# embedded-software-laboratory/p-dmpc

Hardware: NVIDIA B200
Metric: vehicle-plans/sec (higher is better)
Workload: dtype f64

## Files before the change

include/pdmpc_b200.h:

```cpp
#ifndef PDMPC_B200_H
#define PDMPC_B200_H

#include <stddef.h>
#include <stdint.h>

#ifdef __cplusplus
extern "C" {
#endif

#define PDMPC_ABI_VERSION 2

#define PDMPC_AREA_STRIDE 8
#define PDMPC_MAX_HP 16
#define PDMPC_MAX_TRIMS 128
#define PDMPC_MAX_JOINT 4
#define PDMPC_MAX_PRED_LANELETS 8

enum pdmpc_status {
    PDMPC_OK = 0,
    PDMPC_ERR_BAD_INPUT = 1,
    PDMPC_ERR_CUDA = 2,
    PDMPC_ERR_CAPACITY = 3,
    PDMPC_ERR_NO_MPA = 4,
    PDMPC_ERR_ALLOC = 5
// ... 80 lines not shown

int pdmpc_create(int device_id, pdmpc_handle **out);
int pdmpc_destroy(pdmpc_handle *h);
const char *pdmpc_last_error(const pdmpc_handle *h);
int pdmpc_abi_version(void);
int pdmpc_get_hp(const pdmpc_handle *h);

int pdmpc_set_node_capacity(pdmpc_handle *h, int32_t max_nodes_per_search);

int pdmpc_set_variant(pdmpc_handle *h, int32_t variant);

int pdmpc_set_cta_queue(pdmpc_handle *h, int32_t valid_only);

int pdmpc_set_escalation(pdmpc_handle *h, int32_t pops, int32_t short_list_max);

int pdmpc_set_tile_points(pdmpc_handle *h, int32_t points);

int pdmpc_set_cta_heap_smem(pdmpc_handle *h, int32_t entries);

int pdmpc_set_pipeline_chunks(pdmpc_handle *h, int32_t chunks);

int pdmpc_pipeline_bounds(int32_t n_searches, int32_t chunks, int32_t cap, int32_t *bounds, int32_t *n_chunks);

int pdmpc_get_pipeline_timeline(pdmpc_handle *h, int32_t cap, double *host_ms, double *in_ms, double *done_ms, int32_t *n_chunks);

int pdmpc_upload_mpa(pdmpc_handle *h, const pdmpc_mpa_desc *mpa);

int pdmpc_plan_batch(pdmpc_handle *h, const pdmpc_batch_in *in, pdmpc_batch_out *out);

int pdmpc_stage_batch(pdmpc_handle *h, const pdmpc_batch_in *in);
// ... 124 lines not shown
```

p-dmpc_b200/capi.py:

```python
from __future__ import annotations

import ctypes as C
import os
from typing import Optional

import numpy as np

from .mpa import MotionPrimitiveAutomaton
from .records import BatchResult, SearchBatch

_PKG_DIR = os.path.dirname(os.path.abspath(__file__))
LIB_PATH = os.path.join(_PKG_DIR, "csrc", "libpdmpc_b200.so")

PDMPC_OK = 0
PDMPC_ERR_BAD_INPUT = 1
PDMPC_ERR_CUDA = 2
PDMPC_ERR_CAPACITY = 3
PDMPC_ERR_NO_MPA = 4
PDMPC_ERR_ALLOC = 5

EXPORTED_SYMBOLS = (
    "pdmpc_create", "pdmpc_destroy", "pdmpc_last_error", "pdmpc_abi_version",
    "pdmpc_set_node_capacity", "pdmpc_set_variant", "pdmpc_set_tile_points", "pdmpc_set_cta_queue", "pdmpc_set_escalation", "pdmpc_get_hp", "pdmpc_pack_plan_rows", "pdmpc_upload_road", "pdmpc_sample_inputs", "pdmpc_upload_reachable_sets", "pdmpc_assemble_obstacles", "pdmpc_get_pipeline_timeline", "pdmpc_pipeline_bounds", "pdmpc_plan_timestep_from_states", "pdmpc_closed_loop_reset", "pdmpc_plan_timestep_closed_loop", "pdmpc_host_alloc", "pdmpc_host_free",
    "pdmpc_trace_staged", "pdmpc_upload_mpa", "pdmpc_plan_batch", "pdmpc_stage_batch",
    "pdmpc_run_staged", "pdmpc_sync", "pdmpc_fetch_staged", "pdmpc_get_stats", "pdmpc_stream",
    "pdmpc_mcts_plan_batch", "pdmpc_mcts_run_staged", "pdmpc_set_cta_heap_smem", "pdmpc_plan_timestep",
    "pdmpc_set_pipeline_chunks", "pdmpc_measure_fp64_peak", "pdmpc_joint_plan_batch",
)

_p_u8 = C.POINTER(C.c_uint8)
_p_i32 = C.POINTER(C.c_int32)
_p_u64 = C.POINTER(C.c_uint64)
_p_f64 = C.POINTER(C.c_double)


class MpaDesc(C.Structure):
    _fields_ = [
        ("n_trims", C.c_int32), ("Hp", C.c_int32), ("n_edges", C.c_int32),
# ... 180 lines not shown
    lib.pdmpc_get_pipeline_timeline.argtypes = [H, C.c_int32, _p_f64, _p_f64, _p_f64, C.POINTER(C.c_int32)]
    lib.pdmpc_get_pipeline_timeline.restype = C.c_int
    lib.pdmpc_pipeline_bounds.argtypes = [C.c_int32, C.c_int32, C.c_int32, _p_i32, C.POINTER(C.c_int32)]
    lib.pdmpc_pipeline_bounds.restype = C.c_int
    lib.pdmpc_plan_timestep_from_states.argtypes = [H, C.POINTER(TimestepStatesC), C.POINTER(BatchOut)]
    lib.pdmpc_plan_timestep_from_states.restype = C.c_int
    lib.pdmpc_closed_loop_reset.argtypes = [H, C.c_int32, C.c_double, C.c_double]
    lib.pdmpc_closed_loop_reset.restype = C.c_int
    lib.pdmpc_plan_timestep_closed_loop.argtypes = [H, C.POINTER(BatchIn), C.POINTER(TimestepDepsC), _p_i32,
                                                    C.POINTER(C.c_uint8), C.POINTER(BatchOut)]
    lib.pdmpc_plan_timestep_closed_loop.restype = C.c_int
    lib.pdmpc_get_hp.argtypes = [H]
    lib.pdmpc_get_hp.restype = C.c_int
    lib.pdmpc_set_escalation.argtypes = [H, C.c_int32, C.c_int32]
    lib.pdmpc_set_escalation.restype = C.c_int
    lib.pdmpc_set_tile_points.argtypes = [H, C.c_int32]
    lib.pdmpc_set_tile_points.restype = C.c_int
    lib.pdmpc_trace_staged.argtypes = [H, C.c_int32, C.POINTER(C.c_int64), C.c_int64, C.POINTER(C.c_int64)]
    lib.pdmpc_trace_staged.restype = C.c_int
    lib.pdmpc_host_alloc.argtypes = [C.POINTER(C.c_void_p), C.c_size_t]
    lib.pdmpc_host_alloc.restype = C.c_int
    lib.pdmpc_host_free.argtypes = [C.c_void_p]
    lib.pdmpc_host_free.restype = C.c_int
    lib.pdmpc_upload_mpa.argtypes = [H, C.POINTER(MpaDesc)]
    lib.pdmpc_upload_mpa.restype = C.c_int
    lib.pdmpc_plan_batch.argtypes = [H, C.POINTER(BatchIn), C.POINTER(BatchOut)]
    lib.pdmpc_plan_batch.restype = C.c_int
    lib.pdmpc_stage_batch.argtypes = [H, C.POINTER(BatchIn)]
    lib.pdmpc_stage_batch.restype = C.c_int
    lib.pdmpc_run_staged.argtypes = [H]
# ... 160 lines not shown
             "vert_x": np.zeros(vc), "vert_y": np.zeros(vc)}
        ci = CouplingInC(n=n, x=_ptr(x, _p_f64), y=_ptr(y, _p_f64), yaw=_ptr(yaw, _p_f64), speed=_ptr(speed, _p_f64),
                         trim=_ptr(trim, _p_i32), succ_ptr=_ptr(sp, _p_i32), succ_idx=_ptr(si, _p_i32),
                         par_ptr=_ptr(pp, _p_i32), par_idx=_ptr(pi, _p_i32),
                         half_length=float(half_length), half_width=float(half_width))
        oc = ObstaclesOutC(slot_ptr=_ptr(o["slot_ptr"], _p_i32), poly_ptr=_ptr(o["poly_ptr"], _p_i32),
                           vert_x=_ptr(o["vert_x"], _p_f64), vert_y=_ptr(o["vert_y"], _p_f64), poly_capacity=pc, vert_capacity=vc)
        self._check(self.lib.pdmpc_assemble_obstacles(self.h, C.byref(ci), C.byref(oc)))
        o["poly_ptr"] = o["poly_ptr"][: oc.n_polys + 1]
        o["vert_x"], o["vert_y"] = o["vert_x"][: oc.n_verts], o["vert_y"][: oc.n_verts]
        return o

    def set_escalation(self, pops: int, short_list_max: int = -1):
        self._check(self.lib.pdmpc_set_escalation(self.h, int(pops), int(short_list_max)))

    def set_tile_points(self, points: int = 0):
        self._check(self.lib.pdmpc_set_tile_points(self.h, int(points)))

    def trace(self, search: int, cap: int = 1 << 20) -> np.ndarray:
        ids = np.zeros(cap, dtype=np.int64)
        n = C.c_int64()
        self._check(self.lib.pdmpc_trace_staged(self.h, int(search), ids.ctypes.data_as(C.POINTER(C.c_int64)),
                                                cap, C.byref(n)))
        return ids[: min(n.value, cap)].copy()

    def upload_mpa(self, mpa: MotionPrimitiveAutomaton):
        d, keep = mpa_desc(mpa)
        self._check(self.lib.pdmpc_upload_mpa(self.h, C.byref(d)))
        self._mpa_keep = keep
        self._mpa = mpa
# ... 131 lines not shown
```

p-dmpc_b200/csrc/pdmpc_capi.cu:

```cuda
#include <cuda_runtime.h>

#include <algorithm>
#include <cmath>
#include <cstdio>
#include <cstdlib>
#include <cstring>
#include <chrono>
#include <new>
#include <string>
#include <vector>

#include "pdmpc_kernels.cuh"
#include "pdmpc_tiles.cuh"
#include "pdmpc_mcts.cuh"
#include "pdmpc_cta.cuh"
#include "pdmpc_joint.cuh"
#include "pdmpc_inputs.cuh"
#include "pdmpc_fallback.cuh"
#include "pdmpc_obstacles.cuh"

using namespace pdmpc;

namespace {

// ... 27 lines not shown
#ifndef PDMPC_TILE4_PTS
#define PDMPC_TILE4_PTS 256
#endif
constexpr int kTile2Heap = PDMPC_TILE2_HEAP, kTile2Pts = PDMPC_TILE2_PTS, kTile2Ctas = PDMPC_TILE2_CTAS;
constexpr int kTile4Heap = PDMPC_TILE4_HEAP, kTile4Pts = PDMPC_TILE4_PTS, kTile4Ctas = PDMPC_TILE4_CTAS;
#define KERNEL_TILE2 search_tile_kernel<16, kTile2Heap, kTile2Pts, kTile2Ctas>
#define KERNEL_TILE4 search_tile_kernel<8, kTile4Heap, kTile4Pts, kTile4Ctas>
constexpr size_t kTile2Smem = 2 * sizeof(TileSm<kTile2Heap, kTile2Pts>);
constexpr size_t kTile4Smem = 4 * sizeof(TileSm<kTile4Heap, kTile4Pts>);
#ifndef PDMPC_CTA_MASTERS
#define PDMPC_CTA_MASTERS 4
#endif
#ifndef PDMPC_ESCALATE_POPS
#define PDMPC_ESCALATE_POPS 2560
#endif
constexpr int kCtaCheckers = 12;
constexpr int kCtaHeap = 4096, kCtaPts = 512;
constexpr int kCtaMHeap = 1024, kCtaMPts = 256;
constexpr int kCtaMasters = PDMPC_CTA_MASTERS, kCtaMastersDeps = 2;
#define KERNEL_CTA search_cta_kernel<kCtaHeap, kCtaPts, kCtaCheckers, 1, false>
#define KERNEL_CTA_DEPS search_cta_kernel<kCtaHeap, kCtaPts, kCtaCheckers, 1, true>
#define KERNEL_CTAM search_cta_kernel<kCtaMHeap, kCtaMPts, kCtaCheckers, kCtaMasters, false>
#define KERNEL_CTAM_DEPS search_cta_kernel<kCtaMHeap, kCtaMPts, kCtaCheckers, kCtaMastersDeps, true>
using CtaSmemT = CtaSmem<kCtaHeap, kCtaPts, kCtaCheckers, 1, false>;
using CtaDepsSmemT = CtaSmem<kCtaHeap, kCtaPts, kCtaCheckers, 1, true>;
using CtaMSmemT = CtaSmem<kCtaMHeap, kCtaMPts, kCtaCheckers, kCtaMasters, false>;
using CtaMDepsSmemT = CtaSmem<kCtaMHeap, kCtaMPts, kCtaCheckers, kCtaMastersDeps, true>;
static_assert(sizeof(CtaSmemT) <= kSmemLimit && sizeof(CtaDepsSmemT) <= kSmemLimit && sizeof(CtaMSmemT) <= kSmemLimit &&
              sizeof(CtaMDepsSmemT) <= kSmemLimit, "CTA shapes must fit one SM");

// ... 112 lines not shown
    x.a += off; x.b += off; x.cs += off; x.heap += off;
    return x;
}

}

struct pdmpc_handle {
    int device = 0;
    int num_sms = 0;
    int lat_ctas_per_sm = 0;
    int tile_ctas_per_sm[2] = {0, 0};
    int tile_pts_limit = 0;
    int variant_mode = 0;
    int cta_heap_smem = kCtaHeap;
    int escalate_pops = -1;
    int esc_short_list = -1;
    DBuf esc;
    DBuf esc_rows;
    PinnedBuf pin_esc;

    bool cta_valid_only = false;
    bool cta_ok = false;
    bool cta_deps_ok = false;
    DBuf j_veh, j_node, j_heap;
    DBuf d_deps, d_done, d_depx, d_depy, d_depn;
    bool lat_deps_ok = false;
    PinnedBuf pin_deps;
    DepsDev deps{};
    bool deps_staged = false;
    std::vector<int> topo_order;
    cudaStream_t s_in = nullptr, s_out = nullptr, s_comp[7] = {};
// ... 422 lines not shown
    o.n_expanded = reinterpret_cast<int *>(base + h->out_off[2]);
    o.n_pops = reinterpret_cast<int *>(base + h->out_off[3]);
    o.pop_hash = reinterpret_cast<unsigned long long *>(base + h->out_off[4]);
    o.trims = reinterpret_cast<int *>(base + h->out_off[5]);
    o.tree_path = reinterpret_cast<int *>(base + h->out_off[6]);
    o.y_predicted = reinterpret_cast<double *>(base + h->out_off[7]);
    o.g_path = reinterpret_cast<double *>(base + h->out_off[8]);
    o.h_path = reinterpret_cast<double *>(base + h->out_off[9]);
    o.shape_npts = reinterpret_cast<int *>(base + h->out_off[10]);
    o.shape_x = reinterpret_cast<double *>(base + h->out_off[11]);
    o.shape_y = reinterpret_cast<double *>(base + h->out_off[12]);
    o.counters = reinterpret_cast<unsigned long long *>(base + h->out_off[kNumOut]);
    return PDMPC_OK;
}

static void read_counters(pdmpc_handle *h, const unsigned long long counters[16]) {
    h->stats.total_pops = (int64_t)counters[0];
    h->stats.total_nodes = (int64_t)counters[1];
    h->stats.total_obstacle_cols = (int64_t)counters[2];
    if (counters[3]) h->stats.handed_over = (int32_t)counters[3];
    h->stats.escalated = (int32_t)counters[6];
#ifdef PDMPC_PROFILE
    {
#ifdef PDMPC_PROFILE_CHECKER
        static const char *names[8] = {"c:wait_job", "c:tables+place", "c:interx_obstacles", "c:interx_rest", "c:sincos+publish", "-", "-", "c:other"};
#else
        static const char *names[8] = {"setup", "heap_pop", "loads+place", "check", "expand", "heap_push", "wait_children", "loop"};
#endif
        double tot = 0;
        for (int i = 0; i < 8; ++i) tot += (double)counters[8 + i];
        fprintf(stderr, "[pdmpc profile] cycles per pop:");
        for (int i = 0; i < 8; ++i)
            fprintf(stderr, " %s=%.0f", names[i], (double)counters[8 + i] / (double)std::max<unsigned long long>(counters[0], 1));
        fprintf(stderr, " total=%.0f\n", tot / (double)std::max<unsigned long long>(counters[0], 1));
        if (counters[5])
            fprintf(stderr, "[pdmpc profile] checker 0: %.0f cycles per job over %llu jobs\n",
                    (double)counters[4] / (double)counters[5], counters[5]);
    }
#endif
}

static int reserve_polylines(pdmpc_handle *h, int np, int nv, int nl) {
    BatchDev &b = h->batch;
    b.pl_x = b.pl_y = b.ll_x = b.ll_y = nullptr;
    b.pl_xy = b.ll_xy = nullptr;
    if (b.checker != PDMPC_CHECKER_INTERX) return PDMPC_OK;
    CU_TRY(h, h->b_plx.reserve(((size_t)nv + np + 1) * sizeof(double)));
    CU_TRY(h, h->b_ply.reserve(((size_t)nv + np + 1) * sizeof(double)));
    CU_TRY(h, h->b_llx.reserve(((size_t)nl + 2 * b.n + 1) * sizeof(double)));
    CU_TRY(h, h->b_lly.reserve(((size_t)nl + 2 * b.n + 1) * sizeof(double)));
    CU_TRY(h, h->b_plxy.reserve(((size_t)nv + np + 1) * sizeof(double2)));
    CU_TRY(h, h->b_llxy.reserve(((size_t)nl + 2 * b.n + 1) * sizeof(double2)));
    b.pl_x = h->b_plx.as<double>(); b.pl_y = h->b_ply.as<double>();
    b.ll_x = h->b_llx.as<double>(); b.ll_y = h->b_lly.as<double>();
// ... 100 lines not shown
    return stage_finish(h, n, in->checker, in->dt_seconds, dptr, np, nv, nl);
}

static int node_cap(const pdmpc_handle *h) {
    const int cap = h->user_node_cap ? h->user_node_cap : std::min(h->full_tree_nodes + 8, 1 << 20);
    return std::max(std::min(cap, kMaxNodeCap - 1), 64);
}

static bool cta_launchable(const pdmpc_handle *h, bool deps) {
    return (deps ? h->cta_deps_ok : h->cta_ok) && node_cap(h) <= kCtaFlags;
}

static int ensure_arena(pdmpc_handle *h, int slots) {
    const int cap = node_cap(h);
    if (slots <= h->arena_slots && cap == h->arena.cap) return PDMPC_OK;
    slots = std::max(slots, h->arena_slots);
    const size_t tot = (size_t)slots * cap;
    h->arena = ArenaDev{};
    h->arena_slots = 0;
    CU_TRY(h, h->a_a.reserve(tot * sizeof(NodeA)));
    CU_TRY(h, h->a_b.reserve(tot * sizeof(NodeB)));
    CU_TRY(h, h->a_cs.reserve(tot * sizeof(NodeCS)));
    CU_TRY(h, h->a_heap.reserve(tot * sizeof(HEnt)));
    h->arena.a = h->a_a.as<NodeA>();
    h->arena.b = h->a_b.as<NodeB>();
    h->arena.cs = h->a_cs.as<NodeCS>();
    h->arena.heap = h->a_heap.as<HEnt>();
    h->arena.cap = cap;
    h->arena_slots = slots;
    return PDMPC_OK;
}
// ... 25 lines not shown
    else if (shape == kShapeTile4) KERNEL_TILE4<<<grid, kWarp, kTile4Smem, S>>>(h->mpa, bc, h->out, ar, wc, tr, h->tile_pts_limit);
    else KERNEL_LAT<<<grid, kWarp, sizeof(WarpSmem), S>>>(h->mpa, bc, h->out, ar, wc, tr);
    if (cudaGetLastError() != cudaSuccess) return fail(h, PDMPC_ERR_CUDA, "search kernel launch failed");
    h->stats.kernel_launches++;
    return PDMPC_OK;
}

static int escalation_pops(const pdmpc_handle *h, int n) {
    if (h->escalate_pops >= 0) return h->escalate_pops;
    return n >= 300000 ? 4096 : n >= 120000 ? 3072 : PDMPC_ESCALATE_POPS;
}
static bool escalation_on(const pdmpc_handle *h, int shape, int n) {
    return (shape == kShapeTile2 || shape == kShapeTile4) && escalation_pops(h, n) > 0 && cta_launchable(h, false) &&
           n > h->num_sms && h->batch.checker == PDMPC_CHECKER_INTERX;
}

static int escalation_prepare(pdmpc_handle *h, int n, BatchDev *bt, cudaStream_t S) {
    CU_TRY(h, h->esc.reserve(((size_t)n + 4) * sizeof(int)));
    CU_TRY(h, cudaMemsetAsync(h->esc.p, 0, 4 * sizeof(int), S));
    CU_TRY(h, cudaMemsetAsync(h->esc.as<int>() + 4, 0xff, (size_t)n * sizeof(int), S));
    bt->pop_limit = escalation_pops(h, n);
    bt->esc_count = h->esc.as<unsigned>();
    bt->esc_done = h->esc.as<unsigned>() + 1;
    bt->esc_list = h->esc.as<int>() + 4;
    return PDMPC_OK;
}

static int launch_escalated(pdmpc_handle *h, const ArenaDev &ar, int producers, cudaStream_t S) {
    BatchDev be = h->batch;
    be.order = nullptr;
    be.esc_count = h->esc.as<unsigned>();
    be.esc_done = h->esc.as<unsigned>() + 1;
    be.esc_list = h->esc.as<int>() + 4;
    be.esc_producers = (unsigned)producers;
    const int fast = h->cta_valid_only ? 1 : 0;
    unsigned *wc = h->work_counter.as<unsigned>();
    be.esc_gate_lo = 0u; be.esc_gate_hi = (unsigned)(h->esc_short_list >= 0 ? h->esc_short_list : 3 * h->num_sms);
    KERNEL_CTA<<<h->num_sms, CtaShape<1, kCtaCheckers>::kThreads, sizeof(CtaSmemT), S>>>(
        h->mpa, be, h->out, ar, wc + 1, h->cta_heap_smem, fast, DepsDev{});
    be.esc_gate_lo = be.esc_gate_hi; be.esc_gate_hi = 0xffffffffu;
    KERNEL_CTAM<<<h->num_sms, CtaShape<kCtaMasters, kCtaCheckers>::kThreads, sizeof(CtaMSmemT), S>>>(
        h->mpa, be, h->out, ar, wc + 2, h->cta_heap_smem, fast, DepsDev{});
    if (cudaGetLastError() != cudaSuccess) return fail(h, PDMPC_ERR_CUDA, "escalation kernel launch failed");
    h->stats.kernel_launches += 2;
    return PDMPC_OK;
}

static int launch_search(pdmpc_handle *h, const TraceDev &tr) {
    const int n = h->batch.n;
    CU_TRY(h, cudaSetDevice(h->device));
    CU_TRY(h, cudaMemsetAsync(h->out.counters, 0, kCounterBytes, h->stream));
    CU_TRY(h, cudaMemsetAsync(h->work_counter.p, 0, 4 * sizeof(unsigned), h->stream));
    h->stats.handed_over = 0;
    h->stats.escalated = 0;
    h->stats.shape = 0;
    h->batch.hash_valid_only = h->cta_valid_only ? 1 : 0;
    if (n == 0) return PDMPC_OK;
    int shape = h->variant_mode;
    if (shape == kShapeAuto && n <= h->num_sms && tr.search < 0) shape = kShapeCta;
    const bool cta = shape == kShapeCta || shape == kShapeCtaValid;
    if (cta && (!cta_launchable(h, false) || tr.search >= 0)) shape = kShapeLatency;
    if (shape == kShapeCta && h->cta_valid_only) shape = kShapeCtaValid;
    if (shape < kShapeCta) shape = resolve_warp_shape(h, shape, n, h->batch.checker, tr.search >= 0);
    unsigned *wc = h->work_counter.as<unsigned>();
    h->stats.shape = shape;
    if (shape == kShapeCta || shape == kShapeCtaValid) {
        const bool single = n <= h->num_sms;
        const int nm = single ? 1 : kCtaMasters;
        const int grid = std::min((n + nm - 1) / nm, h->num_sms);
        int rc = ensure_arena(h, grid * nm);
        if (rc != PDMPC_OK) return rc;
// ... 4 lines not shown
        else
            KERNEL_CTAM<<<grid, CtaShape<kCtaMasters, kCtaCheckers>::kThreads, sizeof(CtaMSmemT), h->stream>>>(
                h->mpa, h->batch, h->out, h->arena, wc, h->cta_heap_smem, shape == kShapeCtaValid ? 1 : 0, DepsDev{});
        CU_TRY(h, cudaGetLastError());
        h->stats.kernel_launches++;
    } else {
        int slots = 0;
        warp_shape_grid(h, shape, n, &slots);
        const bool esc = escalation_on(h, shape, n) && tr.search < 0;
        int rc = ensure_arena(h, esc ? slots + h->num_sms * kCtaMasters : slots);
        if (rc != PDMPC_OK) return rc;
        BatchDev bt = h->batch;
        if (esc) {
            rc = escalation_prepare(h, n, &bt, h->stream);
            if (rc != PDMPC_OK) return rc;
        }
        CU_TRY(h, cudaEventRecord(h->ev[2], h->stream));
        rc = launch_warp_shape(h, shape, bt, h->arena, wc, tr, h->stream);
        if (rc != PDMPC_OK) return rc;
        if (esc) {
            rc = launch_escalated(h, arena_from(h->arena, slots), warp_shape_grid(h, shape, n), h->stream);
            if (rc != PDMPC_OK) return rc;
        }
    }
    CU_TRY(h, cudaEventRecord(h->ev[3], h->stream));
    h->timing_pending_kernel = true;
    return PDMPC_OK;
}

int pdmpc_run_staged(pdmpc_handle *h) {
    if (!h) return PDMPC_ERR_BAD_INPUT;
    if (!h->staged) return fail(h, PDMPC_ERR_BAD_INPUT, "run_staged: no staged batch");
    TraceDev tr{-1, nullptr, 0, nullptr};
    return launch_search(h, tr);
}

// ... 31 lines not shown
        for (int i = 0; i < kNumOut; ++i)
            if (f.dst[i] && n) memcpy(f.dst[i], src + h->out_off[i], n * f.bytes[i]);
        memcpy(counters, src + h->out_off[kNumOut], sizeof(counters));
        h->stats.d2h_bytes = (int64_t)h->out_bytes;
    } else {
        for (int i = 0; i < kNumOut; ++i)
            if (f.dst[i] && n) {
                CU_TRY(h, cudaMemcpyAsync(f.dst[i], dbase + h->out_off[i], n * f.bytes[i], cudaMemcpyDeviceToHost, h->stream));
                h->stats.d2h_bytes += (int64_t)(n * f.bytes[i]);
            }
        CU_TRY(h, cudaMemcpyAsync(counters, dbase + h->out_off[kNumOut], sizeof(counters), cudaMemcpyDeviceToHost, h->stream));
        CU_TRY(h, cudaEventRecord(h->ev[5], h->stream));
        CU_TRY(h, cudaStreamSynchronize(h->stream));
    }
    h->timing_pending_d2h = true;
    read_counters(h, counters);
    return PDMPC_OK;
}

struct PackDesc {
    const unsigned char *src[kNumOut];
    int bytes[kNumOut], off[kNumOut];
    int row_bytes;
};
__global__ void pack_rows_kernel(PackDesc d, const unsigned *count, const int *list, unsigned char *rows) {
    const unsigned n = *count;
    const int lane = threadIdx.x % 32;
    for (unsigned j = blockIdx.x * (blockDim.x / 32) + threadIdx.x / 32; j < n; j += gridDim.x * (blockDim.x / 32)) {
        const size_t si = (size_t)list[j];
        unsigned char *row = rows + (size_t)j * d.row_bytes;
        for (int f = 0; f < kNumOut; ++f) {
            if (!d.src[f]) continue;
// ... 11 lines not shown
        double v;
        if (o.is_exhausted[r]) {
            v = fb ? fb[(size_t)(r % n_veh) * L + c] : 0.0;
            if (c == 1) v = 1.0;
        } else if (c == 0) v = o.g_path[(size_t)r * (Hp + 1) + Hp];
        else if (c == 1) v = 0.0;
        else if (c < 2 + Hp) v = (double)o.trims[(size_t)r * (Hp + 1) + (c - 2) + 1];
        else if (c < 2 + 4 * Hp) v = o.y_predicted[(size_t)r * Hp * 3 + (c - 2 - Hp)];
        else if (c < 2 + 5 * Hp) v = (double)o.shape_npts[(size_t)r * Hp + (c - 2 - 4 * Hp)];
        else if (c < 2 + 13 * Hp) v = o.shape_x[(size_t)r * Hp * kAreaStride + (c - 2 - 5 * Hp)];
        else v = o.shape_y[(size_t)r * Hp * kAreaStride + (c - 2 - 13 * Hp)];
        dst[idx] = v;
    }
}

int pdmpc_set_escalation(pdmpc_handle *h, int32_t pops, int32_t short_list_max) {
    if (!h) return PDMPC_ERR_BAD_INPUT;
    if (pops < -1) return fail(h, PDMPC_ERR_BAD_INPUT, "escalation threshold must be -1 (by batch size), 0 (off) or a pop count");
    h->escalate_pops = pops;
    h->esc_short_list = short_list_max;
    return PDMPC_OK;
}

constexpr int kPipelineMinSearches = 16384;
constexpr int kPipelineMaxChunks = 16;

static int pipeline_sync_all(pdmpc_handle *h) {
    cudaError_t e = cudaSuccess, e2;
    for (cudaStream_t st : h->s_comp)
        if (st && (e2 = cudaStreamSynchronize(st)) != cudaSuccess) e = e2;
    for (cudaStream_t st : {h->s_in, h->s_out, h->stream})
        if (st && (e2 = cudaStreamSynchronize(st)) != cudaSuccess) e = e2;
    return e == cudaSuccess ? PDMPC_OK : fail(h, PDMPC_ERR_CUDA, std::string("pipeline sync: ") + cudaGetErrorString(e));
}

// ... 148 lines not shown
            d2h_started = true;
        }
        for (int i = 0; i < kNumOut; ++i) {
            if (!f.dst[i]) continue;
            const size_t o0 = (size_t)s0 * f.bytes[i], bytes = (size_t)(s1 - s0) * f.bytes[i];
            if (cudaMemcpyAsync(static_cast<unsigned char *>(f.dst[i]) + o0, dbase + h->out_off[i] + o0, bytes,
                                cudaMemcpyDeviceToHost, h->s_out) != cudaSuccess)
                return bail(fail(h, PDMPC_ERR_CUDA, "pipeline D2H failed"));
            h->stats.d2h_bytes += (int64_t)bytes;
        }
    }
    for (int c = 0; c < C; ++c)
        if (c % lanes != 0 && bnd[c + 1] > bnd[c])
            CU_TRY(h, cudaStreamWaitEvent(h->stream, h->ev_chunk[2 * c + 1], 0));
    if (esc) {
        rc = launch_escalated(h, arena_from(h->arena, (size_t)lanes * slots), esc_producers, h->stream);
        if (rc != PDMPC_OK) return bail(rc);
        CU_TRY(h, cudaMemcpyAsync(h->pin_esc.p, h->esc.p, 4 * sizeof(int), cudaMemcpyDeviceToHost, h->stream));
    }
    CU_TRY(h, cudaEventRecord(h->ev[1], h->s_in));
    CU_TRY(h, cudaEventRecord(h->ev[3], h->stream));
    if (esc) {
        CU_TRY(h, cudaEventRecord(h->ev_fork, h->stream));
        CU_TRY(h, cudaStreamWaitEvent(h->s_out, h->ev_fork, 0));
    }
    unsigned long long counters[16] = {0};
    CU_TRY(h, cudaMemcpyAsync(counters, dbase + h->out_off[kNumOut], sizeof(counters), cudaMemcpyDeviceToHost, h->s_out));
    CU_TRY(h, cudaEventRecord(h->ev[5], h->s_out));
    rc = pipeline_sync_all(h);
    if (rc != PDMPC_OK) return rc;
    if (esc && *h->pin_esc.as<const unsigned>() > 0) {
// ... 16 lines not shown
        CU_TRY(h, cudaGetLastError());
        h->stats.kernel_launches++;
        unsigned char *pin = h->pin_esc.as<unsigned char>();
        CU_TRY(h, cudaMemcpyAsync(pin, h->esc.as<int>() + 4, (size_t)cnt * sizeof(int), cudaMemcpyDeviceToHost, h->stream));
        CU_TRY(h, cudaMemcpyAsync(pin + list_bytes, h->esc_rows.p, (size_t)cnt * off, cudaMemcpyDeviceToHost, h->stream));
        CU_TRY(h, cudaStreamSynchronize(h->stream));
        const int *list = reinterpret_cast<const int *>(pin);
        for (unsigned j = 0; j < cnt; ++j) {
            const unsigned char *row = pin + list_bytes + (size_t)j * off;
            for (int i = 0; i < kNumOut; ++i)
                if (f.dst[i]) memcpy(static_cast<unsigned char *>(f.dst[i]) + (size_t)list[j] * f.bytes[i], row + pd.off[i], f.bytes[i]);
        }
        h->stats.d2h_bytes += (int64_t)(list_bytes + (size_t)cnt * off);
    }
    h->timing_pending_h2d = h->timing_pending_kernel = h->timing_pending_d2h = true;
    read_counters(h, counters);
    h->staged = true;
    return PDMPC_OK;
}

int pdmpc_pipeline_bounds(int32_t n_searches, int32_t chunks, int32_t cap, int32_t *bounds, int32_t *n_chunks) {
    if (n_searches < 2 || chunks < 0 || chunks == 1 || chunks > kPipelineMaxChunks || !bounds || !n_chunks) return PDMPC_ERR_BAD_INPUT;
    const std::vector<int> bnd = pipeline_bounds(n_searches, chunks);
    *n_chunks = (int32_t)bnd.size() - 1;
    if ((int)bnd.size() > cap) return PDMPC_ERR_CAPACITY;
    for (size_t i = 0; i < bnd.size(); ++i) bounds[i] = bnd[i];
    return PDMPC_OK;
}

int pdmpc_get_pipeline_timeline(pdmpc_handle *h, int32_t cap, double *host_ms, double *in_ms, double *done_ms, int32_t *n_chunks) {
    if (!h || !n_chunks) return PDMPC_ERR_BAD_INPUT;
    CU_TRY(h, cudaSetDevice(h->device));
    if (pipeline_sync_all(h) != PDMPC_OK) return PDMPC_ERR_CUDA;
// ... 736 lines not shown
```

p-dmpc_b200/csrc/pdmpc_cta.cuh:

```cuda
#pragma once

#include "pdmpc_kernels.cuh"
#include "pdmpc_tiles.cuh"

namespace pdmpc {

constexpr int kRing = 8;
constexpr int kCtaFlags = 32768;
constexpr int kCtaDepCols = kDepCols;
constexpr int kCtaDepPolys = kCtaDepCols / kAreaStride;

struct __align__(16) CtaJob {
    double px, py, pyaw, c, s;
    unsigned nid0;
    int nchild, sbase, k;
    int terminate;
    int rot;
    int slot;
};

template <int HS, int SP, bool DEPS>
struct __align__(16) CtaSearch {
    double hf[HS + 2];
    unsigned long long hw[HS];
// ... 27 lines not shown
__device__ __forceinline__ void fence_cta() { asm volatile("fence.acq_rel.cta;" ::: "memory"); }

__device__ __forceinline__ void named_bar_sync(int id, int count) {
    asm volatile("bar.sync %0, %1;" ::"r"(id), "r"(count) : "memory");
}
__device__ __forceinline__ void named_bar_arrive(int id, int count) {
    asm volatile("bar.arrive %0, %1;" ::"r"(id), "r"(count) : "memory");
}
__device__ __forceinline__ unsigned flag_get(const volatile unsigned *f, unsigned id) {
    return (f[id >> 4] >> (2u * (id & 15u))) & 3u;
}
__device__ __forceinline__ void flag_set(unsigned *f, unsigned id, unsigned v) {
    atomicOr(f + (id >> 4), v << (2u * (id & 15u)));
}

template <int NM, int NC>
struct CtaShape {
    static constexpr int kParked = NM == 1 ? NC / 3 - 1 : 0;
    static constexpr int kWarps = NM + NC + kParked;
    static constexpr int kThreads = kWarps * kWarp;
    static constexpr int kBarThreads = (NC + 1) * kWarp;
};

template <int HS, int SP, int NC, int NM, bool DEPS = false>
__global__ void __launch_bounds__(CtaShape<NM, NC>::kThreads, 1)
search_cta_kernel(MpaDev m, BatchDev b, OutDev o, ArenaDev ar, unsigned *work_counter, int heap_smem, int fast,
                  DepsDev dp) {
    using Shape = CtaShape<NM, NC>;
    static_assert(NM >= 1 && NC >= 1 && NC <= kWarp, "pool sizes");
    static_assert(NM > 1 || NC % 3 == 0, "single master: three checker warps per scheduler group");
    static_assert(kRing * PDMPC_MAX_TRIMS <= kCtaFlags, "ids in flight");
    constexpr unsigned FULL = 0xffffffffu;
    constexpr int kBarThreads = Shape::kBarThreads;
    extern __shared__ __align__(16) unsigned char smem_raw[];
    CtaSmem<HS, SP, NC, NM, DEPS> &sm = *reinterpret_cast<CtaSmem<HS, SP, NC, NM, DEPS> *>(smem_raw);

    const int warp_id = threadIdx.x / kWarp;
    const int lane = threadIdx.x % kWarp;
    Tile<kWarp> t;
    t.shift = 0; t.lane = lane; t.mask = FULL;
    const int Hp = m.Hp, nT = m.nT;
    volatile unsigned *vdone = sm.done;
    const bool polling = b.esc_producers > 0u;
    if (threadIdx.x < NC) sm.done[threadIdx.x] = 0u;
    if (threadIdx.x == 0) { sm.n_jobs = 0u; sm.rot = 0u; sm.masters_done = 0u; }
    for (int s = 0; s < NM; ++s)
        for (int i = threadIdx.x; i < kCtaFlags / 16; i += Shape::kThreads) sm.S[s].flag2[i] = 0u;
    __syncthreads();

    int role_master = -1, role_checker = -1;
    if (NM == 1) {
        if (warp_id == 0) role_master = 0;
        else if ((warp_id & 3) != 0) role_checker = warp_id - 1 - (warp_id >> 2);
    } else {
        if (warp_id < NM) role_master = warp_id;
        else role_checker = warp_id - NM;
    }
    if (role_master < 0 && role_checker < 0) return;
// ... 203 lines not shown
        bool exact;
        const bool exact_again = redo_exact;
        if (redo_exact) { redo_exact = false; exact = true; }
        else {
            if (!polling) {
                if (lane == 0) si_u = atomicAdd(work_counter, 1u);
                si_u = __shfl_sync(FULL, si_u, 0);
            }
            exact = fast == 0;
        }
        int si;
        if (polling) {
            if (!exact_again) {
                int got = -1;
                if (lane == 0) {
                    const int *cnt = reinterpret_cast<const int *>(b.esc_count);
                    while (ld_acquire_gpu(reinterpret_cast<const int *>(b.esc_done)) < (int)b.esc_producers) __nanosleep(2000);
                    const int total = ld_acquire_gpu(cnt);
                    if ((unsigned)total > b.esc_gate_lo && (unsigned)total <= b.esc_gate_hi) {
                        if (!first_item) next_item = atomicAdd(work_counter, 1u) + gridDim.x * NM;
                        if ((int)next_item < total)
                            while ((got = ld_acquire_gpu(b.esc_list + next_item)) < 0) __nanosleep(200);
                    }
                }
                first_item = false;
                got = __shfl_sync(FULL, got, 0);
                if (got < 0) break;
                si_u = (unsigned)got;
                if (lane == 0 && o.counters) atomicAdd(o.counters + 6, 1ULL);
            }
            si = (int)si_u;
        } else {
            if (si_u >= (unsigned)b.n) break;
            si = b.order ? __ldg(b.order + si_u) : (int)si_u;
        }
        for (int i = lane; i <= clear_upto / 16; i += kWarp) S.flag2[i] = 0u;
        stage_reference(b, si, Hp, S.refx, S.refy, nullptr, t);
        if (lane >= 1 && lane < Hp) {
            double d = 0.0;
            for (int it = 1; it <= Hp - lane; ++it) {
                d = d + b.dt * __ldg(b.v_ref + (size_t)si * Hp + lane + it - 1);
                S.dmax[lane * kMaxHp + it] = d;
            }
        }
// ... 214 lines not shown
            }
            for (int d = 16; d > 0; d >>= 1) extra += __shfl_xor_sync(FULL, extra, d);
            if (__any_sync(FULL, amb)) tie = true;
            n_pops += extra;
        }
        PROF_MARK(7);
        PROF_FLUSH(o, lane == 0);
        clear_upto = n_nodes;
        if (tie) {
            if (lane == 0) atomicAdd(o.counters + 3, 1ULL);
            redo_exact = true;
            continue;
        }
        write_search_result(m, o, na, nb, ncs, S.path, si, trim0, goal, status, exhausted, n_nodes, n_pops, hash, 0ull,
                            true, DEPS ? dp.done : nullptr, t);
    }
    unsigned fin = 0;
    if (lane == 0) fin = atomicAdd(&sm.masters_done, 1u);
    fin = __shfl_sync(FULL, fin, 0);
    if (fin == NM - 1) {
        NodeA z = {0.0, 0.0, 0.0, 0.0};
        publish(z, 0.0, 0.0, 0u, 0, 0, 0, 1);
    }
}

}
```

p-dmpc_b200/csrc/pdmpc_kernels.cuh:

```cuda
#pragma once

#include <cuda_runtime.h>
#include <stdint.h>

#include <cstddef>
#include <type_traits>

#include "../../include/pdmpc_b200.h"

#ifdef PDMPC_PROFILE
#define PROF_DECL long long prof_t0 = clock64(), prof_acc[8] = {0, 0, 0, 0, 0, 0, 0, 0};
#define PROF_MARK(i)                      \
    do {                                  \
        long long _t = clock64();         \
        prof_acc[i] += _t - prof_t0;      \
        prof_t0 = _t;                     \
    } while (0)
#define PROF_FLUSH(o, lane0)                                                              \
    do {                                                                                  \
        if (lane0)                                                                        \
            for (int _i = 0; _i < 8; ++_i) atomicAdd((o).counters + 8 + _i, (unsigned long long)prof_acc[_i]); \
        for (int _i = 0; _i < 8; ++_i) prof_acc[_i] = 0;                                  \
    } while (0)
#else
#define PROF_DECL
#define PROF_MARK(i)
#define PROF_FLUSH(o, lane0)
#endif

namespace pdmpc {

constexpr int kWarp = 32;
constexpr int kAreaStride = PDMPC_AREA_STRIDE;
constexpr int kMaxHp = PDMPC_MAX_HP;
constexpr int kParentCache = 32;

struct MpaDev {
    int nT, Hp, nE;
    const int *succ_ptr;
    const int *succ_te;
    const double *edge_d;
    const int *area_npts;
    const double *area_x, *area_y;
    unsigned bytes_succ_ptr, bytes_succ_te, bytes_edge_d, bytes_area_npts, bytes_area;
    unsigned table_bytes;
    int areas_closed;
};

struct BatchDev {
    int n, checker;
    double dt;
    const int *order;
    int hash_valid_only = 0;
    int pop_limit = 0;
    int *esc_list = nullptr;
    unsigned *esc_count = nullptr, *esc_done = nullptr;
    unsigned esc_producers = 0;
    unsigned esc_gate_lo = 0, esc_gate_hi = 0xffffffffu;
    const double *x0, *y0, *yaw0;
    const int *trim0;
    const double *ref_x, *ref_y, *v_ref;
    const int *slot_ptr, *poly_ptr;
    const double *vert_x, *vert_y;
    const double *pl_x, *pl_y;
    const double2 *pl_xy = nullptr, *ll_xy = nullptr;
    const int *lane_ptr;
    const double *lane_x, *lane_y;
    const double *ll_x, *ll_y;
};

struct OutDev {
    int *status;
    uint8_t *is_exhausted;
// ... 10 lines not shown
    const int *pred_ptr, *pred_idx;
    const int *fb_npts;
    const double *fb_x, *fb_y;
    int *done;
    double *dep_x, *dep_y;
    int *dep_n;
};
constexpr int kDepCols = PDMPC_TIMESTEP_COLS;
__device__ __forceinline__ int ld_acquire_gpu(const int *p) {
    int v;
    asm volatile("ld.acquire.gpu.global.s32 %0, [%1];" : "=r"(v) : "l"(p) : "memory");
    return v;
}
__device__ __forceinline__ void st_release_gpu(int *p, int v) {
    asm volatile("st.release.gpu.global.s32 [%0], %1;" ::"l"(p), "r"(v) : "memory");
}

struct __align__(16) NodeA {
    double x, y, yaw, g;
};
struct __align__(16) NodeB {
    double h;
    unsigned parent;
    unsigned short edge;
    unsigned char trim;
    unsigned char k;
};
struct __align__(16) NodeCS {
    double c, s;
};
// ... 719 lines not shown
```

p-dmpc_b200/csrc/pdmpc_tiles.cuh:

```cuda
#pragma once

#include <type_traits>

#include "pdmpc_kernels.cuh"

namespace pdmpc {

__device__ __forceinline__ unsigned keep_u32(unsigned a) {
    unsigned b;
    asm volatile("mov.u32 %0, %1;" : "=r"(b) : "r"(a));
    return b;
}
__device__ __forceinline__ void sts_f64x2(unsigned a, double x, double y) {
    asm volatile("st.shared.v2.f64 [%0], {%1, %2};" ::"r"(a), "d"(x), "d"(y) : "memory");
}

template <int NE, bool CLOSED>
__device__ __forceinline__ unsigned interx_c2_row(unsigned vb, double dx2, double dy2, double S2) {
    double b[NE + 1];
#pragma unroll
    for (int i = 0; i < NE + (CLOSED ? 0 : 1); ++i) {
        const double2 vv = lds_f64x2(vb + 16u * (unsigned)i);
        b[i] = (vv.y * dx2 - vv.x * dy2) - S2;
    }
// ... 86 lines not shown
            base += TILE;
        }
        if (su && tl == 0) h_st(((p + 1) >> Tt) - 1, v);
        __syncwarp();
    };

    enum { IDLE = 0, RUN = 1, DONE = 2, EXIT = 3 };
    int phase = IDLE;
    int si = 0, trim0 = 0, len = 0;
    const double2 *Op = nullptr, *Lp = nullptr;
    int nlan = 0;
    int n_nodes = 0, n_pops = 0, status = PDMPC_OK;
    unsigned long long hash = 0, cols = 0;
    bool exhausted = false;
    unsigned goal = 0;

    for (;;) {
        if (phase == RUN && b.pop_limit > 0 && n_pops >= b.pop_limit) {
            if (tl == 0) {
                const unsigned q = atomicAdd(b.esc_count, 1u);
                st_release_gpu(b.esc_list + q, si);
            }
            phase = IDLE;
        }
        if (phase == DONE) {
            write_search_result(m, o, na, nb, ncs, sm.path, si, trim0, goal, status, exhausted, n_nodes, n_pops, hash,
                                cols, false, nullptr, t);
            phase = IDLE;
        }
        while (phase == IDLE) {
            unsigned si_u = 0;
            if (tl == 0) si_u = atomicAdd(work_counter, 1u);
            si_u = __shfl_sync(tmask, si_u, shift);
            if (si_u >= (unsigned)b.n) { phase = EXIT; break; }
            si = b.order ? __ldg(b.order + si_u) : (int)si_u;
            __syncwarp(tmask);
            stage_reference(b, si, Hp, sm.refx, sm.refy, sm.vref, t);
            const SearchPolylines pl = search_polylines(b, si, Hp, sm.rng, t);
            const int nl = pl.ll_hi - pl.ll_lo, no = pl.ob_hi - pl.ob_lo;
            const int sp_lim = pts_limit > 0 ? min(pts_limit, SP) : SP;
            const bool lst = nl <= sp_lim, ost = (lst ? nl : 0) + no <= sp_lim;
            if (lst)
                for (int j = tl; j < nl; j += TILE) sm.pts[j] = __ldg(b.ll_xy + pl.ll_lo + j);
            if (ost)
                for (int j = tl; j < no; j += TILE) sm.pts[(lst ? nl : 0) + j] = __ldg(b.pl_xy + pl.ob_lo + j);
            Lp = lst ? sm.pts : b.ll_xy + pl.ll_lo;
            Op = ost ? sm.pts + (lst ? nl : 0) : b.pl_xy + pl.ob_lo;
            nlan = nl;
            trim0 = __ldg(b.trim0 + si);
// ... 289 lines not shown
                HEnt v;
                v.f = __shfl_sync(FULL, he.f, done & (TILE - 1), TILE);
                v.w = __shfl_sync(FULL, he.w, done & (TILE - 1), TILE);
                if (__any_sync(FULL, su)) sift_up_at(su, len, v);
                if (su) { ++len; ++done; }
            }
        }
        if (doexp) n_nodes += nchild;
        __syncwarp();
    }
    if (b.esc_done) {
        __syncwarp();
        __threadfence();
        if (lane == 0) atomicAdd(b.esc_done, 1u);
    }
}

}
```

Baseline: 4.735 million.

## Overlap escalation consumer with tile kernel via PDL and add end-game escalation

The escalation consumer kernel is now launched with programmatic stream serialization, so CTA consumers can start while the warp-tile producers are still running. They pull escalated searches incrementally through a polling take function with a timeout, replacing the two gated consumer launches (short-list CTA plus multi-master) with a single launch. Tile warps also enter an 'end-game' mode once the global work counter is exhausted, and then hand searches over after a lower pop threshold so the long tail moves to the CTA solvers earlier. This risks consumer CTAs spinning and occupying SMs that producers need, and it adds timeline instrumentation that is compiled only under a define.

```diff
diff --git a/include/pdmpc_b200.h b/include/pdmpc_b200.h
--- a/include/pdmpc_b200.h
+++ b/include/pdmpc_b200.h
@@ -118,6 +118,8 @@
 
 int pdmpc_set_escalation(pdmpc_handle *h, int32_t pops, int32_t short_list_max);
 
+int pdmpc_set_endgame_escalation(pdmpc_handle *h, int32_t pops);
+
 int pdmpc_set_tile_points(pdmpc_handle *h, int32_t points);
 
 int pdmpc_set_cta_heap_smem(pdmpc_handle *h, int32_t entries);
diff --git a/p-dmpc_b200/capi.py b/p-dmpc_b200/capi.py
--- a/p-dmpc_b200/capi.py
+++ b/p-dmpc_b200/capi.py
@@ -21,7 +21,7 @@
 
 EXPORTED_SYMBOLS = (
     "pdmpc_create", "pdmpc_destroy", "pdmpc_last_error", "pdmpc_abi_version",
-    "pdmpc_set_node_capacity", "pdmpc_set_variant", "pdmpc_set_tile_points", "pdmpc_set_cta_queue", "pdmpc_set_escalation", "pdmpc_get_hp", "pdmpc_pack_plan_rows", "pdmpc_upload_road", "pdmpc_sample_inputs", "pdmpc_upload_reachable_sets", "pdmpc_assemble_obstacles", "pdmpc_get_pipeline_timeline", "pdmpc_pipeline_bounds", "pdmpc_plan_timestep_from_states", "pdmpc_closed_loop_reset", "pdmpc_plan_timestep_closed_loop", "pdmpc_host_alloc", "pdmpc_host_free",
+    "pdmpc_set_node_capacity", "pdmpc_set_variant", "pdmpc_set_tile_points", "pdmpc_set_cta_queue", "pdmpc_set_escalation", "pdmpc_set_endgame_escalation", "pdmpc_get_hp", "pdmpc_pack_plan_rows", "pdmpc_upload_road", "pdmpc_sample_inputs", "pdmpc_upload_reachable_sets", "pdmpc_assemble_obstacles", "pdmpc_get_pipeline_timeline", "pdmpc_pipeline_bounds", "pdmpc_plan_timestep_from_states", "pdmpc_closed_loop_reset", "pdmpc_plan_timestep_closed_loop", "pdmpc_host_alloc", "pdmpc_host_free",
     "pdmpc_trace_staged", "pdmpc_upload_mpa", "pdmpc_plan_batch", "pdmpc_stage_batch",
     "pdmpc_run_staged", "pdmpc_sync", "pdmpc_fetch_staged", "pdmpc_get_stats", "pdmpc_stream",
     "pdmpc_mcts_plan_batch", "pdmpc_mcts_run_staged", "pdmpc_set_cta_heap_smem", "pdmpc_plan_timestep",
@@ -232,6 +232,8 @@
     lib.pdmpc_get_hp.restype = C.c_int
     lib.pdmpc_set_escalation.argtypes = [H, C.c_int32, C.c_int32]
     lib.pdmpc_set_escalation.restype = C.c_int
+    lib.pdmpc_set_endgame_escalation.argtypes = [H, C.c_int32]
+    lib.pdmpc_set_endgame_escalation.restype = C.c_int
     lib.pdmpc_set_tile_points.argtypes = [H, C.c_int32]
     lib.pdmpc_set_tile_points.restype = C.c_int
     lib.pdmpc_trace_staged.argtypes = [H, C.c_int32, C.POINTER(C.c_int64), C.c_int64, C.POINTER(C.c_int64)]
@@ -422,6 +424,9 @@
     def set_escalation(self, pops: int, short_list_max: int = -1):
         self._check(self.lib.pdmpc_set_escalation(self.h, int(pops), int(short_list_max)))
 
+    def set_endgame_escalation(self, pops: int):
+        self._check(self.lib.pdmpc_set_endgame_escalation(self.h, int(pops)))
+
     def set_tile_points(self, points: int = 0):
         self._check(self.lib.pdmpc_set_tile_points(self.h, int(points)))
 
diff --git a/p-dmpc_b200/csrc/pdmpc_capi.cu b/p-dmpc_b200/csrc/pdmpc_capi.cu
--- a/p-dmpc_b200/csrc/pdmpc_capi.cu
+++ b/p-dmpc_b200/csrc/pdmpc_capi.cu
@@ -65,6 +65,9 @@
 #ifndef PDMPC_ESCALATE_POPS
 #define PDMPC_ESCALATE_POPS 2560
 #endif
+#ifndef PDMPC_ESC_MASTERS
+#define PDMPC_ESC_MASTERS 1
+#endif
 constexpr int kCtaCheckers = 12;
 constexpr int kCtaHeap = 4096, kCtaPts = 512;
 constexpr int kCtaMHeap = 1024, kCtaMPts = 256;
@@ -207,7 +210,7 @@
     int variant_mode = 0;
     int cta_heap_smem = kCtaHeap;
     int escalate_pops = -1;
-    int esc_short_list = -1;
+    int endgame_pops = -1;
     DBuf esc;
     DBuf esc_rows;
     PinnedBuf pin_esc;
@@ -660,7 +663,7 @@
     return PDMPC_OK;
 }
 
-static void read_counters(pdmpc_handle *h, const unsigned long long counters[16]) {
+static int read_counters(pdmpc_handle *h, const unsigned long long counters[16]) {
     h->stats.total_pops = (int64_t)counters[0];
     h->stats.total_nodes = (int64_t)counters[1];
     h->stats.total_obstacle_cols = (int64_t)counters[2];
@@ -684,6 +687,8 @@
                     (double)counters[4] / (double)counters[5], counters[5]);
     }
 #endif
+    if (counters[7]) return fail(h, PDMPC_ERR_CUDA, "escalation consumer: the list's producers did not finish in time");
+    return PDMPC_OK;
 }
 
 static int reserve_polylines(pdmpc_handle *h, int np, int nv, int nl) {
@@ -814,7 +819,7 @@
 static int ensure_arena(pdmpc_handle *h, int slots) {
     const int cap = node_cap(h);
     if (slots <= h->arena_slots && cap == h->arena.cap) return PDMPC_OK;
-    slots = std::max(slots, h->arena_slots);
+    if (cap == h->arena.cap) slots = std::max(slots, h->arena_slots);
     const size_t tot = (size_t)slots * cap;
     h->arena = ArenaDev{};
     h->arena_slots = 0;
@@ -870,6 +875,11 @@
     return (shape == kShapeTile2 || shape == kShapeTile4) && escalation_pops(h, n) > 0 && cta_launchable(h, false) &&
            n > h->num_sms && h->batch.checker == PDMPC_CHECKER_INTERX;
 }
+static int endgame_pops(const pdmpc_handle *h, int n) {
+    if (h->escalate_pops > 0 || h->endgame_pops == 0) return 0;
+    const int e = h->endgame_pops > 0 ? h->endgame_pops : 512;
+    return e < escalation_pops(h, n) ? e : 0;
+}
 
 static int escalation_prepare(pdmpc_handle *h, int n, BatchDev *bt, cudaStream_t S) {
     CU_TRY(h, h->esc.reserve(((size_t)n + 4) * sizeof(int)));
@@ -882,7 +892,7 @@
     return PDMPC_OK;
 }
 
-static int launch_escalated(pdmpc_handle *h, const ArenaDev &ar, int producers, cudaStream_t S) {
+static int launch_escalated(pdmpc_handle *h, const ArenaDev &ar, int producers, cudaStream_t S, bool overlap) {
     BatchDev be = h->batch;
     be.order = nullptr;
     be.esc_count = h->esc.as<unsigned>();
@@ -890,15 +900,23 @@
     be.esc_list = h->esc.as<int>() + 4;
     be.esc_producers = (unsigned)producers;
     const int fast = h->cta_valid_only ? 1 : 0;
-    unsigned *wc = h->work_counter.as<unsigned>();
-    be.esc_gate_lo = 0u; be.esc_gate_hi = (unsigned)(h->esc_short_list >= 0 ? h->esc_short_list : 3 * h->num_sms);
-    KERNEL_CTA<<<h->num_sms, CtaShape<1, kCtaCheckers>::kThreads, sizeof(CtaSmemT), S>>>(
-        h->mpa, be, h->out, ar, wc + 1, h->cta_heap_smem, fast, DepsDev{});
-    be.esc_gate_lo = be.esc_gate_hi; be.esc_gate_hi = 0xffffffffu;
-    KERNEL_CTAM<<<h->num_sms, CtaShape<kCtaMasters, kCtaCheckers>::kThreads, sizeof(CtaMSmemT), S>>>(
-        h->mpa, be, h->out, ar, wc + 2, h->cta_heap_smem, fast, DepsDev{});
-    if (cudaGetLastError() != cudaSuccess) return fail(h, PDMPC_ERR_CUDA, "escalation kernel launch failed");
-    h->stats.kernel_launches += 2;
+    unsigned *wc = h->work_counter.as<unsigned>() + 1;
+    constexpr bool single = PDMPC_ESC_MASTERS == 1;
+    static_assert(single || PDMPC_ESC_MASTERS == PDMPC_CTA_MASTERS, "consumer: 1 or PDMPC_CTA_MASTERS masters per CTA");
+    cudaLaunchAttribute attr[1];
+    attr[0].id = cudaLaunchAttributeProgrammaticStreamSerialization;
+    attr[0].val.programmaticStreamSerializationAllowed = overlap ? 1 : 0;
+    cudaLaunchConfig_t cfg = {};
+    cfg.gridDim = dim3((unsigned)h->num_sms);
+    cfg.blockDim = dim3(single ? CtaShape<1, kCtaCheckers>::kThreads : CtaShape<kCtaMasters, kCtaCheckers>::kThreads);
+    cfg.dynamicSmemBytes = single ? sizeof(CtaSmemT) : sizeof(CtaMSmemT);
+    cfg.stream = S;
+    cfg.attrs = attr;
+    cfg.numAttrs = 1;
+    const cudaError_t e = single ? cudaLaunchKernelEx(&cfg, KERNEL_CTA, h->mpa, be, h->out, ar, wc, h->cta_heap_smem, fast, DepsDev{})
+                                 : cudaLaunchKernelEx(&cfg, KERNEL_CTAM, h->mpa, be, h->out, ar, wc, h->cta_heap_smem, fast, DepsDev{});
+    if (e != cudaSuccess) return fail(h, PDMPC_ERR_CUDA, std::string("escalation kernel launch failed: ") + cudaGetErrorString(e));
+    h->stats.kernel_launches++;
     return PDMPC_OK;
 }
 
@@ -911,6 +929,14 @@
     h->stats.escalated = 0;
     h->stats.shape = 0;
     h->batch.hash_valid_only = h->cta_valid_only ? 1 : 0;
+#ifdef PDMPC_TIMELINE
+    {
+        void *tl = nullptr;
+        CU_TRY(h, cudaGetSymbolAddress(&tl, g_timeline));
+        CU_TRY(h, cudaMemsetAsync(tl, 0, sizeof(Timeline), h->stream));
+        CU_TRY(h, cudaMemsetAsync(tl, 0xff, 4 * sizeof(unsigned long long), h->stream));
+    }
+#endif
     if (n == 0) return PDMPC_OK;
     int shape = h->variant_mode;
     if (shape == kShapeAuto && n <= h->num_sms && tr.search < 0) shape = kShapeCta;
@@ -945,12 +971,13 @@
         if (esc) {
             rc = escalation_prepare(h, n, &bt, h->stream);
             if (rc != PDMPC_OK) return rc;
+            bt.endgame_pops = endgame_pops(h, n);
         }
         CU_TRY(h, cudaEventRecord(h->ev[2], h->stream));
         rc = launch_warp_shape(h, shape, bt, h->arena, wc, tr, h->stream);
         if (rc != PDMPC_OK) return rc;
         if (esc) {
-            rc = launch_escalated(h, arena_from(h->arena, slots), warp_shape_grid(h, shape, n), h->stream);
+            rc = launch_escalated(h, arena_from(h->arena, slots), warp_shape_grid(h, shape, n), h->stream, true);
             if (rc != PDMPC_OK) return rc;
         }
     }
@@ -1012,8 +1039,7 @@
         CU_TRY(h, cudaStreamSynchronize(h->stream));
     }
     h->timing_pending_d2h = true;
-    read_counters(h, counters);
-    return PDMPC_OK;
+    return read_counters(h, counters);
 }
 
 struct PackDesc {
@@ -1055,11 +1081,27 @@
     }
 }
 
-int pdmpc_set_escalation(pdmpc_handle *h, int32_t pops, int32_t short_list_max) {
+int pdmpc_set_escalation(pdmpc_handle *h, int32_t pops, int32_t ) {
     if (!h) return PDMPC_ERR_BAD_INPUT;
     if (pops < -1) return fail(h, PDMPC_ERR_BAD_INPUT, "escalation threshold must be -1 (by batch size), 0 (off) or a pop count");
     h->escalate_pops = pops;
-    h->esc_short_list = short_list_max;
+    return PDMPC_OK;
+}
+
+#ifdef PDMPC_TIMELINE
+int pdmpc_get_timeline(pdmpc_handle *h, void *dst, int64_t bytes) {
+    if (!h || !dst || bytes != (int64_t)sizeof(Timeline)) return PDMPC_ERR_BAD_INPUT;
+    CU_TRY(h, cudaSetDevice(h->device));
+    CU_TRY(h, cudaStreamSynchronize(h->stream));
+    CU_TRY(h, cudaMemcpyFromSymbol(dst, g_timeline, sizeof(Timeline)));
+    return PDMPC_OK;
+}
+#endif
+
+int pdmpc_set_endgame_escalation(pdmpc_handle *h, int32_t pops) {
+    if (!h) return PDMPC_ERR_BAD_INPUT;
+    if (pops < -1) return fail(h, PDMPC_ERR_BAD_INPUT, "end-game threshold must be -1 (by batch size), 0 (off) or a pop count");
+    h->endgame_pops = pops;
     return PDMPC_OK;
 }
 
@@ -1238,7 +1280,7 @@
         if (c % lanes != 0 && bnd[c + 1] > bnd[c])
             CU_TRY(h, cudaStreamWaitEvent(h->stream, h->ev_chunk[2 * c + 1], 0));
     if (esc) {
-        rc = launch_escalated(h, arena_from(h->arena, (size_t)lanes * slots), esc_producers, h->stream);
+        rc = launch_escalated(h, arena_from(h->arena, (size_t)lanes * slots), esc_producers, h->stream, false);
         if (rc != PDMPC_OK) return bail(rc);
         CU_TRY(h, cudaMemcpyAsync(h->pin_esc.p, h->esc.p, 4 * sizeof(int), cudaMemcpyDeviceToHost, h->stream));
     }
@@ -1285,9 +1327,8 @@
         h->stats.d2h_bytes += (int64_t)(list_bytes + (size_t)cnt * off);
     }
     h->timing_pending_h2d = h->timing_pending_kernel = h->timing_pending_d2h = true;
-    read_counters(h, counters);
     h->staged = true;
-    return PDMPC_OK;
+    return read_counters(h, counters);
 }
 
 int pdmpc_pipeline_bounds(int32_t n_searches, int32_t chunks, int32_t cap, int32_t *bounds, int32_t *n_chunks) {
diff --git a/p-dmpc_b200/csrc/pdmpc_cta.cuh b/p-dmpc_b200/csrc/pdmpc_cta.cuh
--- a/p-dmpc_b200/csrc/pdmpc_cta.cuh
+++ b/p-dmpc_b200/csrc/pdmpc_cta.cuh
@@ -65,6 +65,27 @@
     atomicOr(f + (id >> 4), v << (2u * (id & 15u)));
 }
 
+constexpr unsigned long long kEscWaitNs = 30ull * 1000 * 1000 * 1000;
+
+__device__ __forceinline__ int esc_take(const BatchDev &b, unsigned ticket, unsigned long long *err) {
+    const unsigned long long t0 = globaltimer_ns();
+    for (;;) {
+        const bool all_done = ld_acquire_gpu(reinterpret_cast<const int *>(b.esc_done)) >= (int)b.esc_producers;
+        const unsigned count = (unsigned)ld_acquire_gpu(reinterpret_cast<const int *>(b.esc_count));
+        if (ticket < count) {
+            int got;
+            while ((got = ld_acquire_gpu(b.esc_list + ticket)) < 0) {
+                if (globaltimer_ns() - t0 > kEscWaitNs) { if (err) atomicAdd(err, 1ull); return -1; }
+                __nanosleep(200);
+            }
+            return got;
+        }
+        if (all_done) return -1;
+        if (globaltimer_ns() - t0 > kEscWaitNs) { if (err) atomicAdd(err, 1ull); return -1; }
+        __nanosleep(2000);
+    }
+}
+
 template <int NM, int NC>
 struct CtaShape {
     static constexpr int kParked = NM == 1 ? NC / 3 - 1 : 0;
@@ -93,6 +114,7 @@
     const int Hp = m.Hp, nT = m.nT;
     volatile unsigned *vdone = sm.done;
     const bool polling = b.esc_producers > 0u;
+    TIMELINE(if (polling && threadIdx.x == 0) atomicMin(&g_timeline.cons_start, globaltimer_ns());)
     if (threadIdx.x < NC) sm.done[threadIdx.x] = 0u;
     if (threadIdx.x == 0) { sm.n_jobs = 0u; sm.rot = 0u; sm.masters_done = 0u; }
     for (int s = 0; s < NM; ++s)
@@ -326,20 +348,19 @@
             if (!exact_again) {
                 int got = -1;
                 if (lane == 0) {
-                    const int *cnt = reinterpret_cast<const int *>(b.esc_count);
-                    while (ld_acquire_gpu(reinterpret_cast<const int *>(b.esc_done)) < (int)b.esc_producers) __nanosleep(2000);
-                    const int total = ld_acquire_gpu(cnt);
-                    if ((unsigned)total > b.esc_gate_lo && (unsigned)total <= b.esc_gate_hi) {
-                        if (!first_item) next_item = atomicAdd(work_counter, 1u) + gridDim.x * NM;
-                        if ((int)next_item < total)
-                            while ((got = ld_acquire_gpu(b.esc_list + next_item)) < 0) __nanosleep(200);
-                    }
+                    if (!first_item) next_item = atomicAdd(work_counter, 1u) + gridDim.x * NM;
+                    got = esc_take(b, next_item, o.counters ? o.counters + 7 : nullptr);
                 }
                 first_item = false;
                 got = __shfl_sync(FULL, got, 0);
                 if (got < 0) break;
                 si_u = (unsigned)got;
                 if (lane == 0 && o.counters) atomicAdd(o.counters + 6, 1ULL);
+                TIMELINE(if (lane == 0) {
+                    const unsigned long long ts = globaltimer_ns();
+                    atomicMin(&g_timeline.cons_first_item, ts);
+                    if (next_item < (unsigned)kTlItems) g_timeline.item_start[next_item] = ts;
+                })
             }
             si = (int)si_u;
         } else {
@@ -584,6 +605,15 @@
         }
         write_search_result(m, o, na, nb, ncs, S.path, si, trim0, goal, status, exhausted, n_nodes, n_pops, hash, 0ull,
                             true, DEPS ? dp.done : nullptr, t);
+        TIMELINE(if (polling && lane == 0 && next_item < (unsigned)kTlItems) g_timeline.item_end[next_item] = globaltimer_ns();)
+    }
+    if (polling) {
+        asm volatile("griddepcontrol.wait;" ::: "memory");
+        TIMELINE(if (lane == 0) {
+            const unsigned long long te = globaltimer_ns();
+            atomicMax(&g_timeline.cons_end, te);
+            atomicMax(&g_timeline.sm_cons_end[smid_u32() % kTlSms], te);
+        })
     }
     unsigned fin = 0;
     if (lane == 0) fin = atomicAdd(&sm.masters_done, 1u);
diff --git a/p-dmpc_b200/csrc/pdmpc_kernels.cuh b/p-dmpc_b200/csrc/pdmpc_kernels.cuh
--- a/p-dmpc_b200/csrc/pdmpc_kernels.cuh
+++ b/p-dmpc_b200/csrc/pdmpc_kernels.cuh
@@ -30,6 +30,33 @@
 
 namespace pdmpc {
 
+__device__ __forceinline__ unsigned long long globaltimer_ns() {
+    unsigned long long t;
+    asm volatile("mov.u64 %0, %%globaltimer;" : "=l"(t));
+    return t;
+}
+
+#ifdef PDMPC_TIMELINE
+constexpr int kTlSms = 256, kTlItems = 16384;
+struct Timeline {
+    unsigned long long tile_start, exhaust, cons_start, cons_first_item;
+    unsigned long long tile_end, cons_end, esc_mid, esc_endgame;
+    unsigned long long sm_tile_exit[kTlSms];
+    unsigned long long sm_cons_end[kTlSms];
+    unsigned long long item_given_up[kTlItems], item_start[kTlItems], item_end[kTlItems];
+    unsigned item_endgame[kTlItems];
+};
+__device__ Timeline g_timeline;
+__device__ __forceinline__ unsigned smid_u32() {
+    unsigned s;
+    asm volatile("mov.u32 %0, %%smid;" : "=r"(s));
+    return s;
+}
+#define TIMELINE(...) __VA_ARGS__
+#else
+#define TIMELINE(...)
+#endif
+
 constexpr int kWarp = 32;
 constexpr int kAreaStride = PDMPC_AREA_STRIDE;
 constexpr int kMaxHp = PDMPC_MAX_HP;
@@ -53,10 +80,10 @@
     const int *order;
     int hash_valid_only = 0;
     int pop_limit = 0;
+    int endgame_pops = 0;
     int *esc_list = nullptr;
     unsigned *esc_count = nullptr, *esc_done = nullptr;
     unsigned esc_producers = 0;
-    unsigned esc_gate_lo = 0, esc_gate_hi = 0xffffffffu;
     const double *x0, *y0, *yaw0;
     const int *trim0;
     const double *ref_x, *ref_y, *v_ref;
@@ -97,6 +124,11 @@
 }
 __device__ __forceinline__ void st_release_gpu(int *p, int v) {
     asm volatile("st.release.gpu.global.s32 [%0], %1;" ::"l"(p), "r"(v) : "memory");
+}
+__device__ __forceinline__ unsigned ld_relaxed_gpu(const unsigned *p) {
+    unsigned v;
+    asm volatile("ld.relaxed.gpu.global.u32 %0, [%1];" : "=r"(v) : "l"(p) : "memory");
+    return v;
 }
 
 struct __align__(16) NodeA {
diff --git a/p-dmpc_b200/csrc/pdmpc_tiles.cuh b/p-dmpc_b200/csrc/pdmpc_tiles.cuh
--- a/p-dmpc_b200/csrc/pdmpc_tiles.cuh
+++ b/p-dmpc_b200/csrc/pdmpc_tiles.cuh
@@ -124,12 +124,21 @@
     unsigned long long hash = 0, cols = 0;
     bool exhausted = false;
     unsigned goal = 0;
+    bool endgame = false;
+    TIMELINE(if (lane == 0) atomicMin(&g_timeline.tile_start, globaltimer_ns());)
 
     for (;;) {
-        if (phase == RUN && b.pop_limit > 0 && n_pops >= b.pop_limit) {
+        if (phase == RUN && b.endgame_pops > 0 && !endgame && (n_pops & 31) == 0) {
+            unsigned wv = 0;
+            if (tl == 0) wv = ld_relaxed_gpu(work_counter);
+            endgame = __shfl_sync(tmask, wv, shift) >= (unsigned)b.n;
+        }
+        if (phase == RUN && b.pop_limit > 0 && n_pops >= (endgame ? b.endgame_pops : b.pop_limit)) {
             if (tl == 0) {
                 const unsigned q = atomicAdd(b.esc_count, 1u);
                 st_release_gpu(b.esc_list + q, si);
+                TIMELINE(atomicAdd(endgame ? &g_timeline.esc_endgame : &g_timeline.esc_mid, 1ull);
+                         if (q < kTlItems) { g_timeline.item_given_up[q] = globaltimer_ns(); g_timeline.item_endgame[q] = endgame; })
             }
             phase = IDLE;
         }
@@ -142,7 +151,12 @@
             unsigned si_u = 0;
             if (tl == 0) si_u = atomicAdd(work_counter, 1u);
             si_u = __shfl_sync(tmask, si_u, shift);
-            if (si_u >= (unsigned)b.n) { phase = EXIT; break; }
+            if (si_u >= (unsigned)b.n) {
+                asm volatile("griddepcontrol.launch_dependents;" ::: "memory");
+                TIMELINE(if (tl == 0) atomicMin(&g_timeline.exhaust, globaltimer_ns());)
+                phase = EXIT;
+                break;
+            }
             si = b.order ? __ldg(b.order + si_u) : (int)si_u;
             __syncwarp(tmask);
             stage_reference(b, si, Hp, sm.refx, sm.refy, sm.vref, t);
@@ -462,6 +476,11 @@
         __threadfence();
         if (lane == 0) atomicAdd(b.esc_done, 1u);
     }
-}
-
-}
+    TIMELINE(if (lane == 0) {
+        const unsigned long long te = globaltimer_ns();
+        atomicMax(&g_timeline.tile_end, te);
+        atomicMax(&g_timeline.sm_tile_exit[smid_u32() % kTlSms], te);
+    })
+}
+
+}
```

After: 5.007 million, median of 6. 5.8% higher.
